# mengxuyiGit/LGM

Hardware: AMD Instinct MI355X
Metric: Mpixels/s fwd+bwd Gaussian raster (256^2, 100k gauss, 6 views) (higher is better)
Workload: dtype f32

## Files before the change

lgm_amd/build.py:

```python
from __future__ import annotations

import os
import subprocess
import sys

HERE = os.path.dirname(os.path.abspath(__file__))
ROOT = os.path.dirname(HERE)
SOURCES = ["csrc/common.hip", "csrc/render_bin.hip", "csrc/render_raster.hip", "csrc/render_api.hip",
           "csrc/attention.hip", "csrc/head.hip", "csrc/mvattn.hip", "csrc/wgrad.hip"]
FILE_FLAGS = {"csrc/attention.hip": ["-fno-honor-nans"]}
OUT = os.path.join(HERE, "_lib", "liblgm_amd.so")
ARCH = os.environ.get("LGM_AMD_ARCH", "gfx950")
HIPCC = os.environ.get("HIPCC", "/opt/rocm/bin/hipcc")


def sources():
    return [os.path.join(HERE, s) for s in SOURCES if os.path.exists(os.path.join(HERE, s))]


def needs_build() -> bool:
    if not os.path.exists(OUT):
        return True
    t = os.path.getmtime(OUT)
    deps = sources() + [os.path.join(ROOT, "include", f) for f in os.listdir(os.path.join(ROOT, "include"))] + \
        [os.path.join(HERE, "csrc", f) for f in os.listdir(os.path.join(HERE, "csrc")) if f.endswith(".h")]
    return any(os.path.getmtime(p) > t for p in deps)


def build(force: bool = False, verbose: bool = False, out: str = None, defines=()) -> str:
    out = out or OUT
    if out == OUT and not force and not needs_build():
        return OUT
    os.makedirs(os.path.dirname(out), exist_ok=True)
    objs, cmds = [], []
    tag = "" if out == OUT else "." + os.path.basename(out)
    for src in sources():
        obj = os.path.join(HERE, "_lib", os.path.basename(src) + tag + ".o")
        extra = FILE_FLAGS.get(os.path.relpath(src, HERE), [])
        cmd = [HIPCC, f"--offload-arch={ARCH}", "-O3", "-std=c++17", "-fPIC", "-Wall", "-Wno-unused-function",
               "-munsafe-fp-atomics", "-fno-slp-vectorize", "-I", os.path.join(ROOT, "include"), "-I",
               os.path.join(HERE, "csrc"), "-c", src, "-o", obj] + extra + \
            [d if d.startswith("-") else f"-D{d}" for d in defines]
        if verbose:
            print(" ".join(cmd))
        cmds.append(cmd)
        objs.append(obj)
    from concurrent.futures import ThreadPoolExecutor
    with ThreadPoolExecutor(max_workers=min(8, len(cmds))) as ex:
        for r in list(ex.map(lambda c: subprocess.run(c), cmds)):
            if r.returncode:
                raise subprocess.CalledProcessError(r.returncode, r.args)
    tmp = out + ".tmp"
    subprocess.run([HIPCC, f"--offload-arch={ARCH}", "-shared", "-fPIC", "-o", tmp] + objs, check=True)
    os.replace(tmp, out)
    return out


if __name__ == "__main__":
    print(build(force="--force" in sys.argv, verbose=True))
```

lgm_amd/csrc/render_bin.hip:

```cpp
#include "render_common.h"

namespace lgm {
namespace {

enum BinMode { COUNT = 0, EMIT_SLOT = 1, EMIT_PACKED = 2 };

template <int CTRL, int ROW_MASK = 0xf>
__device__ __forceinline__ int dpp_src(int old, int v) {
    return __builtin_amdgcn_update_dpp(old, v, CTRL, ROW_MASK, 0xf, false);
}
__device__ __forceinline__ int wave_incl_scan(int x, int ) {
    x += dpp_src<0x111>(0, x);
    x += dpp_src<0x112>(0, x);
    x += dpp_src<0x114>(0, x);
    x += dpp_src<0x118>(0, x);
    x += dpp_src<0x142, 0xa>(0, x);
    x += dpp_src<0x143, 0xc>(0, x);
    return x;
}

constexpr int BIN_THREADS = 512, BIN_G = BIN_THREADS, BIN_ITERS = 3;
constexpr int BIN_HITCAP = BIN_THREADS * 6;
static_assert(BIN_THREADS <= 512, "owner index packs into 9 bits");

struct BinRec {
    float x, y, kB, k0, k1, dys, mg;
    unsigned c0;
    unsigned cx1;
    unsigned pad_;
    unsigned long long key;
};

__device__ __forceinline__ int wave_incl_max(int v, int ) {
    constexpr int LO = -2147483647 - 1;
    v = max(v, dpp_src<0x111>(LO, v));
    v = max(v, dpp_src<0x112>(LO, v));
    v = max(v, dpp_src<0x114>(LO, v));
    v = max(v, dpp_src<0x118>(LO, v));
    v = max(v, dpp_src<0x142, 0xa>(LO, v));
    v = max(v, dpp_src<0x143, 0xc>(LO, v));
    return v;
}

__device__ void center_order(int gx, int T, int *__restrict__ corder, int *hk) {
    const int gy = (T + gx - 1) / gx, tid = threadIdx.x, w = tid >> 6, lane = tid & 63;
    const int K = min(T, BIN_THREADS);
    const long long maxkey = (long long)(gx - 1) * (gx - 1) + (long long)(gy - 1) * (gy - 1);
    auto key = [&](int t) {
        const int y = t / gx, x = t - y * gx, dx = 2 * x - (gx - 1), dy = 2 * y - (gy - 1);
        return maxkey ? (int)(((long long)dx * dx + (long long)dy * dy) * (K - 1) / maxkey) : 0;
    };
    __syncthreads();
    if (tid < K) hk[tid] = 0;
    __syncthreads();
    for (int t = tid; t < T; t += BIN_THREADS) atomicAdd(&hk[key(t)], 1);
    __syncthreads();
    const int v = tid < K ? hk[tid] : 0;
    const int incl = wave_incl_scan(v, lane);
    if (lane == 63) hk[K + w] = incl;
    __syncthreads();
    int run = incl - v;
    for (int ww = 0; ww < w; ww++) run += hk[K + ww];
    __syncthreads();
    if (tid < K) hk[tid] = run;
    __syncthreads();
    for (int t = tid; t < T; t += BIN_THREADS) corder[atomicAdd(&hk[key(t)], 1)] = t;
}

template <int MODE>
__global__ __launch_bounds__(BIN_THREADS) void k_bin(Dims d, const float *__restrict__ gauss, const float *__restrict__ views,
                                                     const float *__restrict__ projs, float4 *__restrict__ gP,
                                                     float4 *__restrict__ gQ,
                                                     uint2 *__restrict__ rects, int *__restrict__ radii_out,
                                                     int *__restrict__ tile_count, const int *__restrict__ tile_start,
                                                     unsigned long long *__restrict__ pairs, long long slot_stride,
                                                     unsigned long long *__restrict__ misc, float *__restrict__ accum,
                                                     int *__restrict__ corder) {
    extern __shared__ int hist[];
    __shared__ BinRec srec[BIN_THREADS];
    __shared__ int sHead[BIN_THREADS], sExcl[BIN_THREADS];
    __shared__ unsigned sHit[BIN_HITCAP];
    __shared__ unsigned short sRank[BIN_HITCAP];
    __shared__ int s_nhit;
    __shared__ unsigned long long s_tot[2];
    const int T = d.T, tid = threadIdx.x, w = tid >> 6, lane = tid & 63;
    const int vgroups = (d.V + BIN_ITERS - 1) / BIN_ITERS;
    const int b = blockIdx.y / vgroups, vg0 = (blockIdx.y - b * vgroups) * BIN_ITERS;
    int bv = b * d.V + vg0;
    const bool lds = T <= LDS_HIST_MAX;
    int *hbase = hist + T, *fill = hist + 2 * T;
    int *cur = tile_count + (size_t)bv * T;
    if (tid < 2) s_tot[tid] = 0;
    auto dest = [&](int t, int pos) -> long long {
        return (MODE == EMIT_SLOT ? ((long long)bv * T + t) * slot_stride
                                  : (long long)tile_start[(size_t)bv * T + t]) + pos;
    };
    unsigned long long *stamp = d.counters ? d.counters + 8 + 8 * (size_t)d.BV * T +
                                             8 * ((size_t)blockIdx.y * gridDim.x + blockIdx.x)
                                           : nullptr;
    unsigned long long t_ph = 0, ph_acc[3] = {0, 0, 0};
    if (stamp && tid == 0) stamp[0] = t_ph = __builtin_amdgcn_s_memrealtime();
    auto phase = [&](int k) {
        if (stamp && tid == 0) {
            const unsigned long long t = __builtin_amdgcn_s_memrealtime();
            if (k >= 0) ph_acc[k] += t - t_ph;
            t_ph = t;
        }
    };
    const int i = blockIdx.x * BIN_G + tid;
    float g[14];
    if (i < d.N) load_gaussian(gauss + ((size_t)b * d.N + i) * 14, g);
    for (int it = 0; it < BIN_ITERS; it++) {
    if (vg0 + it >= d.V) break;
    bv = b * d.V + vg0 + it;
    cur = tile_count + (size_t)bv * T;
    if (tid == 0) s_nhit = 0;
    if (lds)
        for (int t = tid; t < T; t += BIN_THREADS) hist[t] = 0;
    Geo o;
    bool vis = false;
    if (i < d.N) {
        vis = preprocess_one(g, views + 16 * bv, projs + 16 * bv, d, o);
        if (MODE != COUNT) {
            const size_t k = (size_t)bv * d.N + i;
            if (vis) {
                const float4 rp = rec_p(o.x, o.y, o.A, o.B), rq = rec_q(o.C, o.opacity, o.tau, o.depth);
                gP[k] = rp;
                gQ[k] = rq;
                const bool side = !(d.options & LGM_RENDER_DETERMINISTIC) && rec_needle(rp.z, rp.w, rq.x);
                rects[k] = make_uint2((unsigned)o.x0 | ((unsigned)o.y0 << 16),
                                      (unsigned)o.x1 | ((unsigned)o.y1 << 16) | (side ? 0x80000000u : 0u));
                if (side) {
                    double *sd = reinterpret_cast<double *>(accum + acc_side_offset(d.B, d.V, d.N)) + k * 3;
                    sd[0] = 0.0; sd[1] = 0.0; sd[2] = 0.0;
                }
            } else {
                gP[k] = make_float4(0.f, 0.f, 0.f, 0.f);
                gQ[k] = make_float4(0.f, -INFINITY, -1.f, 0.f);
                rects[k] = make_uint2(0u, 0u);
            }
            if (radii_out) radii_out[k] = vis ? o.radius : 0;
        }
    }
    int nc = 0;
    unsigned long long nref = 0;
    if (vis) {
        BinRec r;
        r.x = o.x; r.y = o.y;
        const float detq = o.A * o.C - o.B * o.B;
        if (o.tau >= 3.0e38f || !(detq > 0.f) || !(o.A > 0.f) || !(o.C > 0.f)) {
            r.kB = 0.f; r.k0 = INFINITY; r.k1 = 0.f; r.dys = 0.f; r.mg = 0.f;
        } else {
            const float iA = __builtin_amdgcn_rcpf(o.A);
            r.kB = o.B * iA;
            r.k0 = fmaxf(o.tau, 0.f) * iA;
            r.k1 = detq * iA * iA;
            const float hxe = sqrtf(fmaxf(o.tau, 0.f) * o.C * __builtin_amdgcn_rcpf(detq));
            r.dys = -o.B * hxe * __builtin_amdgcn_rcpf(o.C);
            r.mg = 1e-3f * hxe + 1e-2f;
        }
        r.c0 = (unsigned)o.cx0 | ((unsigned)o.cy0 << 16);
        r.cx1 = (unsigned)o.cx1;
        r.key = ((unsigned long long)__float_as_uint(o.depth) << 32) | (unsigned)i;
        srec[tid] = r;
        nc = o.cx1 > o.cx0 ? o.cy1 - o.cy0 : 0;
        nref = (unsigned long long)((o.x1 - o.x0) * (o.y1 - o.y0));
    }
#pragma unroll
    for (int o2 = 32; o2 > 0; o2 >>= 1) nref += __shfl_xor(nref, o2, 64);
    if (lane == 0 && nref) atomicAdd(&s_tot[1], nref);
    const int incl = wave_incl_scan(nc, lane), excl = incl - nc;
    const int total = __builtin_amdgcn_readlane(incl, 63);
    sExcl[tid] = excl;
    __syncthreads();
    phase(0);
    unsigned long long nemit = 0;
    auto flat_tests = [&](int pass) {
    int carry = 0;
    for (int base0 = 0; base0 < total; base0 += 64) {
        sHead[tid] = -1;
        __builtin_amdgcn_fence(__ATOMIC_RELEASE, "wavefront");
        if (nc > 0 && excl >= base0 && excl < base0 + 64) sHead[w * 64 + excl - base0] = lane;
        __builtin_amdgcn_fence(__ATOMIC_ACQ_REL, "wavefront");
        int v = sHead[tid];
        if (lane == 0 && v < 0) v = carry;
        v = wave_incl_max(v, lane);
        carry = __builtin_amdgcn_readlane(v, 63);
        const int c = base0 + lane;
        int ta = 0, cnt = 0, trow = 0, owner = 0;
        if (c < total) {
            owner = w * 64 + v;
            const BinRec &e = srec[owner];
            const int ty = (int)(e.c0 >> 16) + (c - sExcl[owner]);
            const float dy0 = (float)(ty * BY) - e.y, dy1 = dy0 + (float)(BY - 1);
            const float e1 = fminf(fmaxf(e.dys, dy0), dy1), e2 = fminf(fmaxf(-e.dys, dy0), dy1);
            const float xh = e.x - e.kB * e1 + sqrtf(fmaxf(e.k0 - e.k1 * e1 * e1, 0.f)) + e.mg;
            const float xl = e.x - e.kB * e2 - sqrtf(fmaxf(e.k0 - e.k1 * e2 * e2, 0.f)) - e.mg;
            const int cx0 = (int)(e.c0 & 0xffffu), cx1 = (int)e.cx1;
            const float fa = ceilf((xl - (float)(BX - 1)) * (1.0f / BX)), fb = floorf(xh * (1.0f / BX)) + 1.f;
            ta = (int)fminf(fmaxf(fa, (float)cx0), (float)cx1);
            const int tb = (int)fminf(fmaxf(fb, (float)ta), (float)cx1);
            cnt = tb - ta;
            trow = ty * d.gx;
        }
        if (pass == 1) {
            for (int k = 0; k < cnt; k++) {
                const int t = trow + ta + k;
                pairs[dest(t, hbase[t] + atomicAdd(&fill[t], 1))] = srec[owner].key;
            }
            continue;
        }
        const int hincl = wave_incl_scan(cnt, lane);
        const int htot = __builtin_amdgcn_readlane(hincl, 63);
        nemit += (unsigned)htot;
        if (!htot) continue;
        if (lds) {
            int slot0 = 0;
            if (MODE != COUNT && lane == 0) slot0 = atomicAdd(&s_nhit, htot);
            slot0 = __builtin_amdgcn_readlane(slot0, 0) + hincl - cnt;
            for (int k = 0; k < cnt; k++) {
                const int t = trow + ta + k;
                const int rk = atomicAdd(&hist[t], 1);
                if (MODE != COUNT) {
                    const int slot = slot0 + k;
                    if (slot < BIN_HITCAP) {
                        sHit[slot] = (unsigned)owner | ((unsigned)t << 9);
                        sRank[slot] = (unsigned short)rk;
                    }
                }
            }
        } else {
            for (int k = 0; k < cnt; k++) {
                const int t = trow + ta + k;
                const int pos = atomicAdd(&cur[t], 1);
                if (MODE != COUNT) pairs[dest(t, pos)] = srec[owner].key;
            }
        }
    }
    };
    flat_tests(0);
    if (lane == 0 && nemit) atomicAdd(&s_tot[0], nemit);
    if (lds) {
        __syncthreads();
        phase(1);
        for (int t = tid; t < T; t += BIN_THREADS) {
            const int c = hist[t];
            if (c) {
                if (MODE == COUNT) atomicAdd(&cur[t], c);
                else hbase[t] = atomicAdd(&cur[t], c);
            }
            fill[t] = 0;
        }
        __syncthreads();
        phase(2);
        if (MODE != COUNT) {
            const int H = s_nhit;
            if (H <= BIN_HITCAP) {
                for (int h = tid; h < H; h += BIN_THREADS) {
                    const unsigned e2 = sHit[h];
                    const int t = (int)(e2 >> 9);
                    pairs[dest(t, hbase[t] + sRank[h])] = srec[e2 & 511u].key;
                }
            } else {
                flat_tests(1);
            }
        }
    }
    __syncthreads();
    phase(-1);
    if (stamp && tid == 0) {
        stamp[1] = ph_acc[0];
        stamp[2] = ph_acc[1];
        stamp[3] = ph_acc[2];
        stamp[4] = t_ph;
        stamp[5] = (unsigned long long)s_nhit;
        stamp[6] = __builtin_amdgcn_s_getreg((31 << 11) | 4);
        stamp[7] = __builtin_amdgcn_s_getreg((3 << 11) | 20);
    }
    }
    if (tid == 0) {
        atomicAdd(&misc[0], s_tot[0]);
        atomicAdd(&misc[1], s_tot[1]);
    }
    if (corder && blockIdx.x == 0 && blockIdx.y == 0) center_order(d.gx, T, corder, hist);
}

__global__ __launch_bounds__(1024) void k_scan(const int *__restrict__ count, int M, int *__restrict__ start) {
    __shared__ long long wsum[16];
    const int tid = threadIdx.x, lane = tid & 63, wid = tid >> 6;
    const int per = (M + 1023) / 1024;
    const int lo = min(M, tid * per), hi = min(M, lo + per);
    long long s = 0;
    for (int i = lo; i < hi; i++) s += count[i];
    long long x = s;
#pragma unroll
    for (int dd = 1; dd < 64; dd <<= 1) {
        const long long y = __shfl_up(x, dd, 64);
        if (lane >= dd) x += y;
    }
    if (lane == 63) wsum[wid] = x;
    __syncthreads();
    if (wid == 0) {
        long long w = lane < 16 ? wsum[lane] : 0;
#pragma unroll
        for (int dd = 1; dd < 16; dd <<= 1) {
            const long long y = __shfl_up(w, dd, 64);
            if (lane >= dd) w += y;
        }
        if (lane < 16) wsum[lane] = w;
    }
    __syncthreads();
    long long run = x - s + (wid > 0 ? wsum[wid - 1] : 0);
    for (int i = lo; i < hi; i++) {
        start[i] = (int)run;
        run += count[i];
    }
    if (tid == 1023) start[M] = (int)wsum[15];
}

constexpr int RS_THREADS = 512, RS_WAVES = RS_THREADS / 64, RS_CAP = 4032,
              RS_MAXR = (RS_CAP + RS_THREADS - 1) / RS_THREADS;
constexpr int RS_OBLK = 4096;
static_assert(RS_CAP <= RS_OBLK && RS_CAP % 64 == 0, "sort image layout");
constexpr int RS_DBITS = 9, RS_B = 1 << RS_DBITS;
typedef unsigned short RsCnt;
constexpr int RS_LDS_LSD = RS_CAP * 4 + RS_CAP * 2 + RS_WAVES * RS_B * (int)sizeof(RsCnt);
constexpr int RS_LDS = RS_LDS_LSD > RS_CAP * 8 + 2048 * 4 ? RS_LDS_LSD : RS_CAP * 8 + 2048 * 4;
static_assert(RS_CAP < 65536, "u16 counters");
static_assert(RS_LDS >= RS_OBLK * 8, "sort_oversized reuses the image as u64[RS_OBLK]");
static_assert(RS_LDS + 512 <= 160 * 1024 / 4, "4 sort workgroups per CU (with the static __shared__ words)");
static_assert(RS_B % RS_THREADS == 0 || RS_THREADS % RS_B == 0, "bucket scan layout");

__device__ __forceinline__ unsigned long long lanemask_lt(int lane) { return (1ull << lane) - 1ull; }

__device__ __forceinline__ unsigned long long match_digit(unsigned dgt, bool valid, int nbits) {
    unsigned long long peers = __ballot(valid);
    for (int b = 0; b < nbits; b++) {
        const bool bit = (dgt >> b) & 1u;
        const unsigned long long m = __ballot(bit);
        peers &= bit ? m : ~m;
    }
    return peers;
}

__device__ __forceinline__ unsigned wave_min_u32(unsigned v) {
#pragma unroll
    for (int o = 32; o > 0; o >>= 1) v = min(v, (unsigned)__shfl_xor((int)v, o, 64));
    return v;
}
__device__ __forceinline__ unsigned wave_max_u32(unsigned v) {
#pragma unroll
    for (int o = 32; o > 0; o >>= 1) v = max(v, (unsigned)__shfl_xor((int)v, o, 64));
    return v;
}

__device__ __forceinline__ void radix_pass(const unsigned (&kr)[RS_MAXR], const unsigned short (&pr)[RS_MAXR],
                                          int shift, int nbits, int n, int c0, int R, unsigned *sk,
                                          unsigned short *sp, RsCnt *cnt, int *s_wsum) {
    const int tid = threadIdx.x, w = tid >> 6, lane = tid & 63;
    const unsigned mask = (1u << nbits) - 1u;
    RsCnt *my = cnt + w * RS_B;
    for (int q = lane; q < RS_B; q += 64) my[q] = 0;
    const unsigned long long lt = lanemask_lt(lane);
    int lr[RS_MAXR];
#pragma unroll
    for (int r = 0; r < RS_MAXR; r++) {
        lr[r] = 0;
        if (r < R) {
            const int e = c0 + r * 64 + lane;
            const bool valid = e < n;
            const unsigned dgt = (kr[r] >> shift) & mask;
            const unsigned long long peers = match_digit(dgt, valid, nbits);
            if (valid) {
                const int rk = __popcll(peers & lt);
                const int b0 = my[dgt];
                lr[r] = b0 + rk;
                if (rk == 0) my[dgt] = (RsCnt)(b0 + __popcll(peers));
            }
        }
    }
    __syncthreads();
    constexpr int BPT = RS_B / RS_THREADS > 0 ? RS_B / RS_THREADS : 1;
    int tot = 0;
    if (tid * BPT < RS_B) {
#pragma unroll
        for (int j = 0; j < BPT; j++)
            for (int ww = 0; ww < RS_WAVES; ww++) tot += cnt[ww * RS_B + tid * BPT + j];
    }
    const int incl = wave_incl_scan(tot, lane);
    if (lane == 63) s_wsum[w] = incl;
    __syncthreads();
    if (tid * BPT < RS_B) {
        int run = incl - tot;
        for (int ww = 0; ww < w; ww++) run += s_wsum[ww];
#pragma unroll
        for (int j = 0; j < BPT; j++)
            for (int ww = 0; ww < RS_WAVES; ww++) {
                const int x = cnt[ww * RS_B + tid * BPT + j];
                cnt[ww * RS_B + tid * BPT + j] = (RsCnt)run;
                run += x;
            }
    }
    __syncthreads();
#pragma unroll
    for (int r = 0; r < RS_MAXR; r++) {
        if (r < R) {
            const int e = c0 + r * 64 + lane;
            if (e < n) {
                const int pos = my[(kr[r] >> shift) & mask] + lr[r];
                sk[pos] = kr[r];
                sp[pos] = pr[r];
            }
        }
    }
    __syncthreads();
}

__device__ __forceinline__ void cas64(unsigned long long *s, int lo, int hi) {
    const unsigned long long a = s[lo], b = s[hi];
    if (a > b) { s[lo] = b; s[hi] = a; }
}

__device__ void sort_oversized(unsigned long long *seg, int n, unsigned long long *sk) {
    const int C = RS_OBLK;
    int m = 1;
    while (m < n) m <<= 1;
    for (int c0 = 0; c0 < n; c0 += C) {
        const int nb = min(C, n - c0);
        for (int q = threadIdx.x; q < nb; q += blockDim.x) sk[q] = seg[c0 + q];
        __syncthreads();
        for (int k = 2; k <= C; k <<= 1) {
            for (int p = threadIdx.x; p < (C >> 1); p += blockDim.x) {
                const int half = k >> 1, lo = (p / half) * k + (p % half), hi = lo ^ (k - 1);
                if (hi < nb) cas64(sk, lo, hi);
            }
            __syncthreads();
            for (int j = k >> 2; j > 0; j >>= 1) {
// ... 160 lines not shown
        vall = max(vall, s_wmm[2][ww]);
    }
    if (tid == 0) s_vmax = vall;
    const unsigned span = kmax - kmin;
    const int kbits = span ? 32 - __clz(span) : 0;
#pragma unroll
    for (int r = 0; r < RS_MAXR; r++) kr[r] -= kmin;
    auto reload = [&]() {
#pragma unroll
        for (int r = 0; r < RS_MAXR; r++) {
            if (r < R) {
                const int e = c0 + r * 64 + lane;
                if (e < n) { kr[r] = sk[e]; pr[r] = sp[e]; }
            }
        }
    };
    if (kbits > 0 && msd_sort(kr, ir, n, c0, R, kbits, sk, reinterpret_cast<unsigned *>(smem) + 2 * RS_CAP, s_wsum,
                              &s_flag, reinterpret_cast<unsigned *>(seg)))
        return;
    unsigned idr[RS_MAXR];
#pragma unroll
    for (int r = 0; r < RS_MAXR; r++) pr[r] = (unsigned short)(c0 + r * 64 + lane);
    for (int sh = 0; sh < kbits; sh += RS_DBITS) {
        radix_pass(kr, pr, sh, min(RS_DBITS, kbits - sh), n, c0, R, sk, sp, cnt, s_wsum);
        reload();
    }
    if (kbits == 0) {
#pragma unroll
        for (int r = 0; r < RS_MAXR; r++) {
            if (r < R) {
                const int e = c0 + r * 64 + lane;
                if (e < n) { sk[e] = kr[r]; sp[e] = pr[r]; }
            }
        }
        __syncthreads();
    }
    for (int q = tid + 32; q < n; q += RS_THREADS)
        if (sk[q] == sk[q - 32]) s_long = 1;
    __syncthreads();
    if (s_long) {
#pragma unroll
        for (int r = 0; r < RS_MAXR; r++) {
            const int e = c0 + r * 64 + lane;
            if (r < R && e < n) { kr[r] = (unsigned)seg[e]; pr[r] = (unsigned short)e; }
        }
        const int vbits = s_vmax ? 32 - __clz(s_vmax) : 0;
        for (int sh = 0; sh < vbits; sh += RS_DBITS) {
            radix_pass(kr, pr, sh, min(RS_DBITS, vbits - sh), n, c0, R, sk, sp, cnt, s_wsum);
            reload();
        }
#pragma unroll
        for (int r = 0; r < RS_MAXR; r++) {
            const int e = c0 + r * 64 + lane;
            if (r < R && e < n) kr[r] = (unsigned)(seg[pr[r]] >> 32) - kmin;
        }
        for (int sh = 0; sh < kbits; sh += RS_DBITS) {
            radix_pass(kr, pr, sh, min(RS_DBITS, kbits - sh), n, c0, R, sk, sp, cnt, s_wsum);
            reload();
        }
#pragma unroll
        for (int r = 0; r < RS_MAXR; r++) {
            idr[r] = 0u;
            const int e = c0 + r * 64 + lane;
            if (r < R && e < n) idr[r] = (unsigned)seg[pr[r]];
        }
    } else {
#pragma unroll
        for (int r = 0; r < RS_MAXR; r++) {
            idr[r] = 0u;
            const int e = c0 + r * 64 + lane;
            if (r < R && e < n) idr[r] = (unsigned)seg[sp[e]];
        }
        bool any_tie = false;
        for (int q = tid; q + 1 < n; q += RS_THREADS) any_tie |= sk[q] == sk[q + 1];
        if (__syncthreads_or(any_tie)) {
            unsigned *ids_l = reinterpret_cast<unsigned *>(sp);
#pragma unroll
            for (int r = 0; r < RS_MAXR; r++) {
                const int e = c0 + r * 64 + lane;
                if (r < R && e < n) ids_l[e] = idr[r];
            }
            __syncthreads();
            for (int q = tid; q < n; q += RS_THREADS) {
                if (q + 1 < n && sk[q] == sk[q + 1] && (q == 0 || sk[q - 1] != sk[q])) {
                    int e = q + 1;
                    while (e < n && sk[e] == sk[q]) e++;
                    for (int a2 = q + 1; a2 < e; a2++) {
                        const unsigned v = ids_l[a2];
                        int z = a2 - 1;
                        while (z >= q && ids_l[z] > v) { ids_l[z + 1] = ids_l[z]; z--; }
                        ids_l[z + 1] = v;
                    }
                }
            }
            __syncthreads();
#pragma unroll
            for (int r = 0; r < RS_MAXR; r++) {
                const int e = c0 + r * 64 + lane;
                if (r < R && e < n) idr[r] = ids_l[e];
            }
        }
    }
    __syncthreads();
    unsigned *ids = reinterpret_cast<unsigned *>(seg);
#pragma unroll
    for (int r = 0; r < RS_MAXR; r++) {
        const int e = c0 + r * 64 + lane;
        if (r < R && e < n) ids[e] = idr[r];
    }
}

__global__ __launch_bounds__(RS_THREADS) __attribute__((amdgpu_waves_per_eu(8))) void k_sort(
    int M, long long slot_stride, const int *__restrict__ tile_start, const int *__restrict__ tile_count,
    unsigned long long *__restrict__ pairs, unsigned long long *__restrict__ counters, int BV, int T,
    const int *__restrict__ corder) {
    int tile = xcd_item(blockIdx.x, M);
    if (corder) {
        const int r = (int)blockIdx.x / BV, v = (int)blockIdx.x - r * BV;
        tile = v * T + corder[r];
    }
    long long base;
    int n;
    tile_range(tile, slot_stride, tile_start, tile_count, base, n);
    const unsigned long long t_start = __builtin_amdgcn_s_memrealtime();
    if (counters && threadIdx.x == 0) {
        counters[8 + 8 * (size_t)tile + 4] = t_start;
        counters[8 + 8 * (size_t)tile + 6] = (unsigned long long)n;
    }
    sort_tile(base, n, pairs);
    if (counters) {
        __syncthreads();
        if (threadIdx.x == 0) counters[8 + 8 * (size_t)tile + 5] = __builtin_amdgcn_s_memrealtime();
    }
}

}

int launch_binning(const Dims &d, const float *gaussians, const float *cam_view, const float *cam_view_proj,
                   char *ws, const Layout &L, int *radii_out, long long *stats_out, bool count_only,
                   hipStream_t st) {
    const size_t M = (size_t)d.BV * d.T;
    if (hipMemsetAsync(ws + L.tile_count, 0, L.misc + 64 - L.tile_count, st) != hipSuccess) {
        set_error("hipMemsetAsync failed");
        return LGM_E_HIP;
    }
    float4 *gP = (float4 *)(ws + L.gP), *gQ = (float4 *)(ws + L.gQ);
    uint2 *rects = (uint2 *)(ws + L.rects);
    int *tcount = (int *)(ws + L.tile_count), *tstart = (int *)(ws + L.tile_start);
    unsigned long long *pairs = (unsigned long long *)(ws + L.pairs), *misc = (unsigned long long *)(ws + L.misc);
    float *accum = (float *)(ws + L.accum);
    const size_t lds = d.T <= LDS_HIST_MAX ? 3 * (size_t)d.T * 4 : 0;
    int *corder = lds && d.T >= 8 ? (int *)(ws + L.order) : nullptr;
    dim3 grid((d.N + BIN_G - 1) / BIN_G, d.B * ((d.V + BIN_ITERS - 1) / BIN_ITERS));
    if (d.N > 0) {
        if (count_only || !L.slot) {
            LGM_LAUNCH("k_bin_count", st, (k_bin<COUNT><<<grid, BIN_THREADS, lds, st>>>(d, gaussians, cam_view, cam_view_proj,
                       gP, gQ, rects, nullptr, tcount, tstart, pairs, 0, misc, accum, nullptr)));
        }
        if (!count_only) {
            if (L.slot) {
                LGM_LAUNCH("k_bin", st, (k_bin<EMIT_SLOT><<<grid, BIN_THREADS, lds, st>>>(d, gaussians, cam_view, cam_view_proj,
                           gP, gQ, rects, radii_out, tcount, tstart, pairs, (long long)d.N, misc, accum, corder)));
            } else {
                LGM_LAUNCH("k_scan", st, (k_scan<<<1, 1024, 0, st>>>(tcount, (int)M, tstart)));
                if (hipMemsetAsync(ws + L.tile_count, 0, L.misc + 64 - L.tile_count, st) != hipSuccess) {
                    set_error("hipMemsetAsync failed");
                    return LGM_E_HIP;
                }
                LGM_LAUNCH("k_bin", st, (k_bin<EMIT_PACKED><<<grid, BIN_THREADS, lds, st>>>(d, gaussians, cam_view,
                           cam_view_proj, gP, gQ, rects, radii_out, tcount, tstart, pairs, 0, misc, accum, corder)));
            }
            LGM_LAUNCH("k_sort", st, (k_sort<<<(unsigned)M, RS_THREADS, RS_LDS, st>>>(
                                         (int)M, L.slot ? (long long)d.N : -1LL, tstart, tcount, pairs, d.counters,
                                         d.BV, d.T, corder)));
        }
    }
    if (d.N == 0 && !L.slot && hipMemsetAsync(ws + L.tile_start, 0, (M + 1) * 4, st) != hipSuccess) {
        set_error("hipMemsetAsync failed");
        return LGM_E_HIP;
    }
    if (stats_out && hipMemcpyAsync(stats_out, ws + L.misc, 16, hipMemcpyDeviceToDevice, st) != hipSuccess) {
        set_error("hipMemcpyAsync failed");
        return LGM_E_HIP;
    }
    return LGM_OK;
}

}
```

lgm_amd/csrc/render_common.h:

```cpp
#pragma once
#include <hip/hip_runtime.h>
#include <stdint.h>

#include "common.h"
#include "lgm_render.h"

namespace lgm {

constexpr int BX = 16, BY = 16, TILE_PIX = BX * BY;
constexpr int NACC = 10;
constexpr int NACC_V = 6, NACC_S = 4;
__host__ __device__ __forceinline__ size_t acc_index(int q, size_t bvN_i, size_t bN_i, size_t BVN) {
    return q < 5 ? bvN_i * NACC_V + q : q < 9 ? BVN * NACC_V + bN_i * NACC_S + (q - 5) : bvN_i * NACC_V + 5;
}
__host__ __device__ inline size_t acc_elems(size_t B, size_t V, size_t N) { return B * V * N * NACC_V + B * N * NACC_S; }
__host__ __device__ inline size_t acc_side_offset(size_t B, size_t V, size_t N) { return (acc_elems(B, V, N) + 1) & ~(size_t)1; }
__host__ __device__ inline int det_flush_limit_log2(int V, int T, bool scene_record) {
    const long long f = scene_record ? (long long)V * T : (long long)T;
    int c = 0;
    while ((1ll << c) < f) c++;
    return 62 - c;
}
constexpr int LDS_HIST_MAX = 8192;
constexpr float LOG2E = 1.4426950408889634f;
// ... 47 lines not shown
    L.cmask = take(BV * P);
    L.accum = take(det ? acc_elems(B, V, N) * 8 : acc_side_offset(B, V, N) * 4 + BV * N * 3 * 8);
    L.lossp = take(BV * T * 2 * 4);
    L.lossw = take(((BV * T + 2047) / 2048) * 16);
    L.detmax = take(64 * 4);
    L.total = o;
    return L;
}

struct Dims {
    int B, V, N, H, W, gx, gy, T, BV;
    float tanx, tany, fx, fy, mod;
    unsigned long long *counters;
    int det_lim_log2;
    int options;
    int ck_shift;
    const float *gt_img, *gt_mask;
    float *loss_part;
    float *loss_out;
    const float *d_loss;
};

__device__ __forceinline__ void xf43(const float *M, float x, float y, float z, float o[3]) {
#pragma clang fp contract(off)
    o[0] = M[0] * x + M[4] * y + M[8] * z + M[12];
    o[1] = M[1] * x + M[5] * y + M[9] * z + M[13];
    o[2] = M[2] * x + M[6] * y + M[10] * z + M[14];
}
__device__ __forceinline__ void xf44(const float *M, float x, float y, float z, float o[4]) {
#pragma clang fp contract(off)
    o[0] = M[0] * x + M[4] * y + M[8] * z + M[12];
    o[1] = M[1] * x + M[5] * y + M[9] * z + M[13];
    o[2] = M[2] * x + M[6] * y + M[10] * z + M[14];
    o[3] = M[3] * x + M[7] * y + M[11] * z + M[15];
}

__device__ __forceinline__ void quat_rot(const float q[4], float R[3][3]) {
#pragma clang fp contract(off)
    const float r = q[0], x = q[1], y = q[2], z = q[3];
    R[0][0] = 1.f - 2.f * (y * y + z * z); R[0][1] = 2.f * (x * y - r * z); R[0][2] = 2.f * (x * z + r * y);
    R[1][0] = 2.f * (x * y + r * z); R[1][1] = 1.f - 2.f * (x * x + z * z); R[1][2] = 2.f * (y * z - r * x);
    R[2][0] = 2.f * (x * z - r * y); R[2][1] = 2.f * (y * z + r * x); R[2][2] = 1.f - 2.f * (x * x + y * y);
}

__device__ __forceinline__ void cov3d(const float s[3], const float R[3][3], float c3[6]) {
#pragma clang fp contract(off)
    float M[3][3];
#pragma unroll
    for (int c = 0; c < 3; c++)
#pragma unroll
        for (int k = 0; k < 3; k++) M[c][k] = s[k] * R[c][k];
#define LGM_SIG(c, r) (M[r][0] * M[c][0] + M[r][1] * M[c][1] + M[r][2] * M[c][2])
    c3[0] = LGM_SIG(0, 0); c3[1] = LGM_SIG(0, 1); c3[2] = LGM_SIG(0, 2);
    c3[3] = LGM_SIG(1, 1); c3[4] = LGM_SIG(1, 2); c3[5] = LGM_SIG(2, 2);
#undef LGM_SIG
}

struct ProjCtx {
    float T0[3], T1[3];
    float t[3];
    float xmul, ymul;
};
__device__ __forceinline__ ProjCtx make_proj(const float *Vw, float mx, float my, float mz, float fx, float fy,
                                             float tanx, float tany) {
#pragma clang fp contract(off)
    ProjCtx P;
    xf43(Vw, mx, my, mz, P.t);
    const float limx = 1.3f * tanx, limy = 1.3f * tany;
    const float txtz = P.t[0] / P.t[2], tytz = P.t[1] / P.t[2];
    P.t[0] = fminf(limx, fmaxf(-limx, txtz)) * P.t[2];
    P.t[1] = fminf(limy, fmaxf(-limy, tytz)) * P.t[2];
    P.xmul = (txtz < -limx || txtz > limx) ? 0.f : 1.f;
    P.ymul = (tytz < -limy || tytz > limy) ? 0.f : 1.f;
    const float tz = P.t[2];
    const float J00 = fx / tz, J02 = -(fx * P.t[0]) / (tz * tz);
    const float J11 = fy / tz, J12 = -(fy * P.t[1]) / (tz * tz);
#pragma unroll
    for (int r = 0; r < 3; r++) {
        P.T0[r] = Vw[4 * r + 0] * J00 + Vw[4 * r + 2] * J02;
        P.T1[r] = Vw[4 * r + 1] * J11 + Vw[4 * r + 2] * J12;
    }
    return P;
}
__device__ __forceinline__ void cov2d(const ProjCtx &P, const float c3[6], float &a, float &b, float &c) {
#pragma clang fp contract(off)
    const float S[3][3] = {{c3[0], c3[1], c3[2]}, {c3[1], c3[3], c3[4]}, {c3[2], c3[4], c3[5]}};
    float s0[3], s1[3];
#pragma unroll
    for (int k = 0; k < 3; k++) {
        s0[k] = S[k][0] * P.T0[0] + S[k][1] * P.T0[1] + S[k][2] * P.T0[2];
        s1[k] = S[k][0] * P.T1[0] + S[k][1] * P.T1[1] + S[k][2] * P.T1[2];
    }
    a = P.T0[0] * s0[0] + P.T0[1] * s0[1] + P.T0[2] * s0[2] + 0.3f;
    b = s1[0] * P.T0[0] + s1[1] * P.T0[1] + s1[2] * P.T0[2];
    c = P.T1[0] * s1[0] + P.T1[1] * s1[1] + P.T1[2] * s1[2] + 0.3f;
}

__device__ __forceinline__ float ndc2pix(float v, int S) { return (float)((((double)v + 1.0) * S - 1.0) * 0.5); }

__device__ __forceinline__ bool ellipse_hits_rect(float x, float y, float A, float B, float C, float invA,
                                                  float invC, float tau, float rx0, float rx1, float ry0, float ry1) {
    if (tau >= 3.0e38f) return true;
    if (x >= rx0 && x <= rx1 && y >= ry0 && y <= ry1) return true;
    float best = 3.0e38f;
    const float ex[2] = {rx0, rx1}, ey[2] = {ry0, ry1};
#pragma unroll
    for (int e = 0; e < 2; e++) {
        const float dx = x - ex[e];
        const float dy = fminf(fmaxf(-B * dx * invC, y - ry1), y - ry0);
        best = fminf(best, A * dx * dx + 2.f * B * dx * dy + C * dy * dy);
    }
#pragma unroll
    for (int e = 0; e < 2; e++) {
        const float dy = y - ey[e];
        const float dx = fminf(fmaxf(-B * dy * invA, x - rx1), x - rx0);
        best = fminf(best, A * dx * dx + 2.f * B * dx * dy + C * dy * dy);
    }
    return best <= tau;
}

constexpr float KQ = 0.5f * LOG2E;
__device__ __forceinline__ float4 rec_p(float x, float y, float A, float B) {
    return make_float4(x, y, -KQ * A, -LOG2E * B);
}
__device__ __forceinline__ float4 rec_q(float C, float opacity, float tau, float depth) {
    return make_float4(-KQ * C, opacity > 0.f ? log2f(opacity) : -INFINITY, tau >= 3.0e38f ? tau : KQ * tau, depth);
}
__device__ __forceinline__ bool rec_needle(float Ap, float Bp, float Cp) {
#pragma clang fp contract(off)
    const float sac = Ap + Cp, dq = Ap * Cp - 0.25f * Bp * Bp;
    return !(sac * sac <= ACC_NEEDLE * dq);
}
__device__ __forceinline__ bool rec_hits_rect(const float4 &p, const float4 &q, float rx0, float rx1, float ry0,
                                              float ry1) {
    const float A = -p.z, B = -0.5f * p.w, C = -q.x;
    return ellipse_hits_rect(p.x, p.y, A, B, C, 1.0f / A, 1.0f / C, q.z, rx0, rx1, ry0, ry1);
}
__device__ __forceinline__ void rec_conic(const float4 &p, const float4 &q, float &A, float &B, float &C, float &op) {
    A = p.z * (-1.0f / KQ);
    B = p.w * (-1.0f / LOG2E);
    C = q.x * (-1.0f / KQ);
    op = exp2f(q.y);
}

struct Geo {
    float x, y, depth, A, B, C, opacity;
    float hx, hy;
    float tau;
    int x0, y0, x1, y1;
    int cx0, cy0, cx1, cy1;
    int radius;
};

__device__ __forceinline__ bool preprocess_one(const float *g, const float *Vw, const float *Pm, const Dims &d,
                                               Geo &o) {
#pragma clang fp contract(off)
    float hom[4], pv[3];
    xf44(Pm, g[0], g[1], g[2], hom);
    const float pw = 1.0f / (hom[3] + 0.0000001f);
    const float ppx = hom[0] * pw, ppy = hom[1] * pw;
    xf43(Vw, g[0], g[1], g[2], pv);
    if (pv[2] <= 0.2f) return false;
    float R[3][3];
    const float q[4] = {g[7], g[8], g[9], g[10]};
    quat_rot(q, R);
    const float s[3] = {d.mod * g[4], d.mod * g[5], d.mod * g[6]};
    float c3[6];
    cov3d(s, R, c3);
    const ProjCtx P = make_proj(Vw, g[0], g[1], g[2], d.fx, d.fy, d.tanx, d.tany);
    float a, b, c;
    cov2d(P, c3, a, b, c);
    const float det = a * c - b * b;
    if (det == 0.0f) return false;
    const float det_inv = 1.f / det;
    const float mid = 0.5f * (a + c);
    const float l1 = mid + sqrtf(fmaxf(0.1f, mid * mid - det));
    const float l2 = mid - sqrtf(fmaxf(0.1f, mid * mid - det));
    const float rad = ceilf(3.f * sqrtf(fmaxf(l1, l2)));
    const float px = ndc2pix(ppx, d.W), py = ndc2pix(ppy, d.H);
    const int r = (int)rad;
    const int x0 = min(d.gx, max(0, (int)((px - r) / BX)));
    const int y0 = min(d.gy, max(0, (int)((py - r) / BY)));
    const int x1 = min(d.gx, max(0, (int)((px + r + BX - 1) / BX)));
    const int y1 = min(d.gy, max(0, (int)((py + r + BY - 1) / BY)));
    if ((x1 - x0) * (y1 - y0) == 0) return false;
    o.x = px; o.y = py; o.depth = pv[2];
    o.A = c * det_inv; o.B = -b * det_inv; o.C = a * det_inv;
    o.opacity = g[3];
    o.x0 = x0; o.y0 = y0; o.x1 = x1; o.y1 = y1; o.radius = r;
    const float op = g[3];
    if (d.options & LGM_RENDER_NO_CULL) {
        o.hx = o.hy = 3.0e38f;
        o.tau = 3.0e38f;
        o.cx0 = x0; o.cx1 = x1; o.cy0 = y0; o.cy1 = y1;
        return true;
    }
    if (!(op * 255.0f > 1.0f)) {
        o.hx = o.hy = -1.f;
        o.tau = -1.f;
        o.cx0 = o.cx1 = x0; o.cy0 = o.cy1 = y0;
        return true;
    }
    const float cond = (a + c) * (a + c) * __builtin_amdgcn_rcpf(det);
    if (!(det > 0.f) || !(cond < 4e4f)) {
        o.hx = o.hy = 3.0e38f;
        o.tau = 3.0e38f;
        o.cx0 = x0; o.cx1 = x1; o.cy0 = y0; o.cy1 = y1;
        return true;
    }
    const float tau = (2.0f * 0.6931471805599453f) * __builtin_amdgcn_logf(255.0f * op) * (1.001f + 2e-5f * cond) + 1e-3f;
    o.tau = tau;
    o.hx = sqrtf(tau * fmaxf(a, 0.f));
    o.hy = sqrtf(tau * fmaxf(c, 0.f));
    const float lx = fmaxf(-1.0f, fminf((float)d.gx, (px - o.hx - (BX - 1)) / BX));
    const float hxt = fmaxf(-1.0f, fminf((float)d.gx, (px + o.hx) / BX));
    const float ly = fmaxf(-1.0f, fminf((float)d.gy, (py - o.hy - (BY - 1)) / BY));
    const float hyt = fmaxf(-1.0f, fminf((float)d.gy, (py + o.hy) / BY));
    o.cx0 = max(x0, (int)ceilf(lx));
    o.cx1 = min(x1, (int)floorf(hxt) + 1);
    o.cy0 = max(y0, (int)ceilf(ly));
    o.cy1 = min(y1, (int)floorf(hyt) + 1);
    if (o.cx1 < o.cx0) o.cx1 = o.cx0;
    if (o.cy1 < o.cy0) o.cy1 = o.cy0;
    return true;
}

__device__ __forceinline__ void load_gaussian(const float *__restrict__ src, float g[14]) {
    const float2 *p = reinterpret_cast<const float2 *>(src);
#pragma unroll
    for (int k = 0; k < 7; k++) {
        const float2 v = p[k];
        g[2 * k] = v.x;
        g[2 * k + 1] = v.y;
    }
}

__device__ __forceinline__ void tile_range(int tile, long long slot_stride, const int *__restrict__ tile_start,
                                           const int *__restrict__ tile_count, long long &base, int &n) {
    if (slot_stride >= 0) {
        base = (long long)tile * slot_stride;
        n = tile_count[tile];
    } else {
        base = tile_start[tile];
        n = tile_start[tile + 1] - tile_start[tile];
    }
}

__host__ __device__ __forceinline__ int xcd_item(int b, int M) {
    const int q = M >> 3, r = M & 7, g = b & 7, i = b >> 3;
    return (g < r ? g * (q + 1) : r * (q + 1) + (g - r) * q) + i;
}
__host__ __device__ __forceinline__ int xcd_group(int t, int M) {
    const int q = M >> 3, r = M & 7;
    return t < r * (q + 1) ? t / (q + 1) : r + (t - r * (q + 1)) / (q > 0 ? q : 1);
}
__host__ __device__ __forceinline__ int round8(int x) { return (x + 7) & ~7; }

__device__ __forceinline__ void tile_pixel(int t, int &lx, int &ly) {
    const int w = t >> 6, l = t & 63;
    lx = ((w & 1) << 3) + (l & 7);
    ly = ((w >> 1) << 3) + (l >> 3);
}

int launch_binning(const Dims &d, const float *gaussians, const float *cam_view, const float *cam_view_proj,
                   char *ws, const Layout &L, int *radii_out, long long *stats_out, bool count_only,
                   hipStream_t st);
int launch_render_fwd(const Dims &d, const float *gaussians, const float *bg, float *image, float *depth,
                      float *alpha, char *ws, const Layout &L, hipStream_t st);
int launch_loss_reduce(const Dims &d, char *ws, const Layout &L, hipStream_t st);
int launch_render_bwd(const Dims &d, const float *gaussians, const float *cam_view, const float *cam_view_proj,
                      const float *bg, const float *d_image, const float *d_depth, const float *d_alpha,
                      float *d_gaussians, float *d_means2D, char *ws, const Layout &L, hipStream_t st);

}
```

Baseline: 2569.

## Specialize binning kernel on stats/stamps, hoist cov3d, pack hit rank

The binning kernel is templated on whether statistics and timing stamps are needed, so the default path drops the reduction atomics and the stamp bookkeeping. The 3D covariance is computed once per gaussian outside the per-view loop, and only the position is reloaded per view. The per-hit rank is packed into the same 32-bit word as the owner and tile, which removes a shared array. A waves-per-EU attribute is also set to cap register pressure. Together these aim to cut VGPR and LDS use and redundant work, at the cost of more kernel instantiations.

```diff
diff --git a/lgm_amd/build.py b/lgm_amd/build.py
--- a/lgm_amd/build.py
+++ b/lgm_amd/build.py
@@ -27,6 +27,14 @@
     return any(os.path.getmtime(p) > t for p in deps)
 
 
+def compile_cmd(src: str, obj: str, defines=()) -> list:
+    extra = FILE_FLAGS.get(os.path.relpath(src, HERE), [])
+    return [HIPCC, f"--offload-arch={ARCH}", "-O3", "-std=c++17", "-fPIC", "-Wall", "-Wno-unused-function",
+            "-munsafe-fp-atomics", "-fno-slp-vectorize", "-I", os.path.join(ROOT, "include"), "-I",
+            os.path.join(HERE, "csrc"), "-c", src, "-o", obj] + extra + \
+        [d if d.startswith("-") else f"-D{d}" for d in defines]
+
+
 def build(force: bool = False, verbose: bool = False, out: str = None, defines=()) -> str:
     out = out or OUT
     if out == OUT and not force and not needs_build():
@@ -36,11 +44,7 @@
     tag = "" if out == OUT else "." + os.path.basename(out)
     for src in sources():
         obj = os.path.join(HERE, "_lib", os.path.basename(src) + tag + ".o")
-        extra = FILE_FLAGS.get(os.path.relpath(src, HERE), [])
-        cmd = [HIPCC, f"--offload-arch={ARCH}", "-O3", "-std=c++17", "-fPIC", "-Wall", "-Wno-unused-function",
-               "-munsafe-fp-atomics", "-fno-slp-vectorize", "-I", os.path.join(ROOT, "include"), "-I",
-               os.path.join(HERE, "csrc"), "-c", src, "-o", obj] + extra + \
-            [d if d.startswith("-") else f"-D{d}" for d in defines]
+        cmd = compile_cmd(src, obj, defines)
         if verbose:
             print(" ".join(cmd))
         cmds.append(cmd)
diff --git a/lgm_amd/csrc/render_bin.hip b/lgm_amd/csrc/render_bin.hip
--- a/lgm_amd/csrc/render_bin.hip
+++ b/lgm_amd/csrc/render_bin.hip
@@ -21,7 +21,12 @@
 
 constexpr int BIN_THREADS = 512, BIN_G = BIN_THREADS, BIN_ITERS = 3;
 constexpr int BIN_HITCAP = BIN_THREADS * 6;
-static_assert(BIN_THREADS <= 512, "owner index packs into 9 bits");
+static_assert(BIN_THREADS <= 512, "owner index and tile rank pack into 9 bits each");
+static_assert(LDS_HIST_MAX <= 1 << 13, "the tile index of a hit packs into 13 bits");
+#ifndef LGM_BIN_WAVES
+#define LGM_BIN_WAVES 6
+#endif
+constexpr int bin_waves(bool stats) { return stats ? 4 : LGM_BIN_WAVES; }
 
 struct BinRec {
     float x, y, kB, k0, k1, dys, mg;
@@ -67,20 +72,17 @@
     for (int t = tid; t < T; t += BIN_THREADS) corder[atomicAdd(&hk[key(t)], 1)] = t;
 }
 
-template <int MODE>
-__global__ __launch_bounds__(BIN_THREADS) void k_bin(Dims d, const float *__restrict__ gauss, const float *__restrict__ views,
-                                                     const float *__restrict__ projs, float4 *__restrict__ gP,
-                                                     float4 *__restrict__ gQ,
-                                                     uint2 *__restrict__ rects, int *__restrict__ radii_out,
-                                                     int *__restrict__ tile_count, const int *__restrict__ tile_start,
-                                                     unsigned long long *__restrict__ pairs, long long slot_stride,
-                                                     unsigned long long *__restrict__ misc, float *__restrict__ accum,
-                                                     int *__restrict__ corder) {
+template <int MODE, bool STATS, bool STAMPS>
+__global__ __launch_bounds__(BIN_THREADS) __attribute__((amdgpu_waves_per_eu(bin_waves(STATS)))) void k_bin(
+    Dims d, const float *__restrict__ gauss, const float *__restrict__ views, const float *__restrict__ projs,
+    float4 *__restrict__ gP, float4 *__restrict__ gQ, uint2 *__restrict__ rects, int *__restrict__ radii_out,
+    int *__restrict__ tile_count, const int *__restrict__ tile_start, unsigned long long *__restrict__ pairs,
+    long long slot_stride, unsigned long long *__restrict__ misc, float *__restrict__ accum,
+    int *__restrict__ corder) {
     extern __shared__ int hist[];
     __shared__ BinRec srec[BIN_THREADS];
     __shared__ int sHead[BIN_THREADS], sExcl[BIN_THREADS];
     __shared__ unsigned sHit[BIN_HITCAP];
-    __shared__ unsigned short sRank[BIN_HITCAP];
     __shared__ int s_nhit;
     __shared__ unsigned long long s_tot[2];
     const int T = d.T, tid = threadIdx.x, w = tid >> 6, lane = tid & 63;
@@ -90,26 +92,37 @@
     const bool lds = T <= LDS_HIST_MAX;
     int *hbase = hist + T, *fill = hist + 2 * T;
     int *cur = tile_count + (size_t)bv * T;
-    if (tid < 2) s_tot[tid] = 0;
+    if constexpr (STATS)
+        if (tid < 2) s_tot[tid] = 0;
     auto dest = [&](int t, int pos) -> long long {
         return (MODE == EMIT_SLOT ? ((long long)bv * T + t) * slot_stride
                                   : (long long)tile_start[(size_t)bv * T + t]) + pos;
     };
-    unsigned long long *stamp = d.counters ? d.counters + 8 + 8 * (size_t)d.BV * T +
-                                             8 * ((size_t)blockIdx.y * gridDim.x + blockIdx.x)
-                                           : nullptr;
-    unsigned long long t_ph = 0, ph_acc[3] = {0, 0, 0};
-    if (stamp && tid == 0) stamp[0] = t_ph = __builtin_amdgcn_s_memrealtime();
+    __shared__ unsigned long long s_ph[4];
+    unsigned long long *stamp = nullptr;
+    if constexpr (STAMPS) {
+        stamp = d.counters + 8 + 8 * (size_t)d.BV * T + 8 * ((size_t)blockIdx.y * gridDim.x + blockIdx.x);
+        if (tid == 0) {
+            s_ph[0] = s_ph[1] = s_ph[2] = 0;
+            stamp[0] = s_ph[3] = __builtin_amdgcn_s_memrealtime();
+        }
+    }
     auto phase = [&](int k) {
-        if (stamp && tid == 0) {
-            const unsigned long long t = __builtin_amdgcn_s_memrealtime();
-            if (k >= 0) ph_acc[k] += t - t_ph;
-            t_ph = t;
+        if constexpr (STAMPS) {
+            if (tid == 0) {
+                const unsigned long long t = __builtin_amdgcn_s_memrealtime();
+                if (k >= 0) s_ph[k] += t - s_ph[3];
+                s_ph[3] = t;
+            }
         }
     };
     const int i = blockIdx.x * BIN_G + tid;
-    float g[14];
-    if (i < d.N) load_gaussian(gauss + ((size_t)b * d.N + i) * 14, g);
+    float c3[6];
+    if (i < d.N) {
+        float g[14];
+        load_gaussian(gauss + ((size_t)b * d.N + i) * 14, g);
+        gaussian_cov3d(g, d.mod, c3);
+    }
     for (int it = 0; it < BIN_ITERS; it++) {
     if (vg0 + it >= d.V) break;
     bv = b * d.V + vg0 + it;
@@ -120,7 +133,10 @@
     Geo o;
     bool vis = false;
     if (i < d.N) {
-        vis = preprocess_one(g, views + 16 * bv, projs + 16 * bv, d, o);
+        const float2 *gp = reinterpret_cast<const float2 *>(gauss + ((size_t)b * d.N + i) * 14);
+        const float2 g01 = gp[0], g23 = gp[1];
+        const float gm[4] = {g01.x, g01.y, g23.x, g23.y};
+        vis = preprocess_view(gm, c3, views + 16 * bv, projs + 16 * bv, d, o);
         if (MODE != COUNT) {
             const size_t k = (size_t)bv * d.N + i;
             if (vis) {
@@ -164,11 +180,13 @@
         r.key = ((unsigned long long)__float_as_uint(o.depth) << 32) | (unsigned)i;
         srec[tid] = r;
         nc = o.cx1 > o.cx0 ? o.cy1 - o.cy0 : 0;
-        nref = (unsigned long long)((o.x1 - o.x0) * (o.y1 - o.y0));
-    }
-#pragma unroll
-    for (int o2 = 32; o2 > 0; o2 >>= 1) nref += __shfl_xor(nref, o2, 64);
-    if (lane == 0 && nref) atomicAdd(&s_tot[1], nref);
+        if constexpr (STATS) nref = (unsigned long long)((o.x1 - o.x0) * (o.y1 - o.y0));
+    }
+    if constexpr (STATS) {
+#pragma unroll
+        for (int o2 = 32; o2 > 0; o2 >>= 1) nref += __shfl_xor(nref, o2, 64);
+        if (lane == 0 && nref) atomicAdd(&s_tot[1], nref);
+    }
     const int incl = wave_incl_scan(nc, lane), excl = incl - nc;
     const int total = __builtin_amdgcn_readlane(incl, 63);
     sExcl[tid] = excl;
@@ -212,7 +230,7 @@
         }
         const int hincl = wave_incl_scan(cnt, lane);
         const int htot = __builtin_amdgcn_readlane(hincl, 63);
-        nemit += (unsigned)htot;
+        if constexpr (STATS) nemit += (unsigned)htot;
         if (!htot) continue;
         if (lds) {
             int slot0 = 0;
@@ -223,10 +241,7 @@
                 const int rk = atomicAdd(&hist[t], 1);
                 if (MODE != COUNT) {
                     const int slot = slot0 + k;
-                    if (slot < BIN_HITCAP) {
-                        sHit[slot] = (unsigned)owner | ((unsigned)t << 9);
-                        sRank[slot] = (unsigned short)rk;
-                    }
+                    if (slot < BIN_HITCAP) sHit[slot] = (unsigned)owner | ((unsigned)rk << 9) | ((unsigned)t << 18);
                 }
             }
         } else {
@@ -239,7 +254,8 @@
     }
     };
     flat_tests(0);
-    if (lane == 0 && nemit) atomicAdd(&s_tot[0], nemit);
+    if constexpr (STATS)
+        if (lane == 0 && nemit) atomicAdd(&s_tot[0], nemit);
     if (lds) {
         __syncthreads();
         phase(1);
@@ -258,8 +274,8 @@
             if (H <= BIN_HITCAP) {
                 for (int h = tid; h < H; h += BIN_THREADS) {
                     const unsigned e2 = sHit[h];
-                    const int t = (int)(e2 >> 9);
-                    pairs[dest(t, hbase[t] + sRank[h])] = srec[e2 & 511u].key;
+                    const int t = (int)(e2 >> 18);
+                    pairs[dest(t, hbase[t] + (int)((e2 >> 9) & 511u))] = srec[e2 & 511u].key;
                 }
             } else {
                 flat_tests(1);
@@ -268,21 +284,27 @@
     }
     __syncthreads();
     phase(-1);
-    if (stamp && tid == 0) {
-        stamp[1] = ph_acc[0];
-        stamp[2] = ph_acc[1];
-        stamp[3] = ph_acc[2];
-        stamp[4] = t_ph;
+    if (STAMPS && tid == 0) {
+        stamp[1] = s_ph[0];
+        stamp[2] = s_ph[1];
+        stamp[3] = s_ph[2];
+        stamp[4] = s_ph[3];
         stamp[5] = (unsigned long long)s_nhit;
         stamp[6] = __builtin_amdgcn_s_getreg((31 << 11) | 4);
         stamp[7] = __builtin_amdgcn_s_getreg((3 << 11) | 20);
     }
     }
-    if (tid == 0) {
+    if (STATS && tid == 0) {
         atomicAdd(&misc[0], s_tot[0]);
         atomicAdd(&misc[1], s_tot[1]);
     }
     if (corder && blockIdx.x == 0 && blockIdx.y == 0) center_order(d.gx, T, corder, hist);
+}
+
+template <int MODE>
+auto bin_kernel(bool stats, bool stamps) {
+    return stats ? (stamps ? k_bin<MODE, true, true> : k_bin<MODE, true, false>)
+                 : (stamps ? k_bin<MODE, false, true> : k_bin<MODE, false, false>);
 }
 
 __global__ __launch_bounds__(1024) void k_scan(const int *__restrict__ count, int M, int *__restrict__ start) {
@@ -749,23 +771,27 @@
     const size_t lds = d.T <= LDS_HIST_MAX ? 3 * (size_t)d.T * 4 : 0;
     int *corder = lds && d.T >= 8 ? (int *)(ws + L.order) : nullptr;
     dim3 grid((d.N + BIN_G - 1) / BIN_G, d.B * ((d.V + BIN_ITERS - 1) / BIN_ITERS));
+    const bool stats = stats_out != nullptr || count_only, stamps = d.counters != nullptr;
     if (d.N > 0) {
         if (count_only || !L.slot) {
-            LGM_LAUNCH("k_bin_count", st, (k_bin<COUNT><<<grid, BIN_THREADS, lds, st>>>(d, gaussians, cam_view, cam_view_proj,
-                       gP, gQ, rects, nullptr, tcount, tstart, pairs, 0, misc, accum, nullptr)));
+            LGM_LAUNCH("k_bin_count", st, (bin_kernel<COUNT>(stats, stamps)<<<grid, BIN_THREADS, lds, st>>>(
+                       d, gaussians, cam_view, cam_view_proj, gP, gQ, rects, nullptr, tcount, tstart, pairs, 0, misc,
+                       accum, nullptr)));
         }
         if (!count_only) {
             if (L.slot) {
-                LGM_LAUNCH("k_bin", st, (k_bin<EMIT_SLOT><<<grid, BIN_THREADS, lds, st>>>(d, gaussians, cam_view, cam_view_proj,
-                           gP, gQ, rects, radii_out, tcount, tstart, pairs, (long long)d.N, misc, accum, corder)));
+                LGM_LAUNCH("k_bin", st, (bin_kernel<EMIT_SLOT>(stats, stamps)<<<grid, BIN_THREADS, lds, st>>>(
+                           d, gaussians, cam_view, cam_view_proj, gP, gQ, rects, radii_out, tcount, tstart, pairs,
+                           (long long)d.N, misc, accum, corder)));
             } else {
                 LGM_LAUNCH("k_scan", st, (k_scan<<<1, 1024, 0, st>>>(tcount, (int)M, tstart)));
                 if (hipMemsetAsync(ws + L.tile_count, 0, L.misc + 64 - L.tile_count, st) != hipSuccess) {
                     set_error("hipMemsetAsync failed");
                     return LGM_E_HIP;
                 }
-                LGM_LAUNCH("k_bin", st, (k_bin<EMIT_PACKED><<<grid, BIN_THREADS, lds, st>>>(d, gaussians, cam_view,
-                           cam_view_proj, gP, gQ, rects, radii_out, tcount, tstart, pairs, 0, misc, accum, corder)));
+                LGM_LAUNCH("k_bin", st, (bin_kernel<EMIT_PACKED>(stats, stamps)<<<grid, BIN_THREADS, lds, st>>>(
+                           d, gaussians, cam_view, cam_view_proj, gP, gQ, rects, radii_out, tcount, tstart, pairs, 0,
+                           misc, accum, corder)));
             }
             LGM_LAUNCH("k_sort", st, (k_sort<<<(unsigned)M, RS_THREADS, RS_LDS, st>>>(
                                          (int)M, L.slot ? (long long)d.N : -1LL, tstart, tcount, pairs, d.counters,
diff --git a/lgm_amd/csrc/render_common.h b/lgm_amd/csrc/render_common.h
--- a/lgm_amd/csrc/render_common.h
+++ b/lgm_amd/csrc/render_common.h
@@ -223,8 +223,16 @@
     int radius;
 };
 
-__device__ __forceinline__ bool preprocess_one(const float *g, const float *Vw, const float *Pm, const Dims &d,
-                                               Geo &o) {
+__device__ __forceinline__ void gaussian_cov3d(const float *g, float mod, float c3[6]) {
+#pragma clang fp contract(off)
+    float R[3][3];
+    const float q[4] = {g[7], g[8], g[9], g[10]};
+    quat_rot(q, R);
+    const float s[3] = {mod * g[4], mod * g[5], mod * g[6]};
+    cov3d(s, R, c3);
+}
+__device__ __forceinline__ bool preprocess_view(const float *g, const float c3[6], const float *Vw, const float *Pm,
+                                                const Dims &d, Geo &o) {
 #pragma clang fp contract(off)
     float hom[4], pv[3];
     xf44(Pm, g[0], g[1], g[2], hom);
@@ -232,12 +240,6 @@
     const float ppx = hom[0] * pw, ppy = hom[1] * pw;
     xf43(Vw, g[0], g[1], g[2], pv);
     if (pv[2] <= 0.2f) return false;
-    float R[3][3];
-    const float q[4] = {g[7], g[8], g[9], g[10]};
-    quat_rot(q, R);
-    const float s[3] = {d.mod * g[4], d.mod * g[5], d.mod * g[6]};
-    float c3[6];
-    cov3d(s, R, c3);
     const ProjCtx P = make_proj(Vw, g[0], g[1], g[2], d.fx, d.fy, d.tanx, d.tany);
     float a, b, c;
     cov2d(P, c3, a, b, c);
```

After: 2621, median of 6. 1.02x the previous value.
